# delldu/TransMVSNet

Hardware: AMD Instinct MI355X
Metric: depth maps/sec @ DTU 864x1152 N=5 (48/32/8 hyp); Abs depth L1 vs ref (higher is better)
Workload: dtype f32; 1 GPU; DTU 864x1152, N=5 views, cascade 48/32/8, B=1, hot path from FeatureNet outputs (FMT+pathway+stage glue+cost volume+CostRegNet+softmax/WTA); global_batch=1, parallelism=replica1, launch=hip_graph replay

## Files before the change

transmvsnet_amd/csrc/costreg.hip:

```cpp
#include "common.h"

namespace tmvs {

typedef float floatx4 __attribute__((ext_vector_type(4)));

template <int N>
struct VecN;
template <>
struct VecN<4> {
  float v[4];
  __device__ __forceinline__ void load(const float* p) {
    const float4 t = *reinterpret_cast<const float4*>(p);
    v[0] = t.x;
    v[1] = t.y;
    v[2] = t.z;
    v[3] = t.w;
  }
  __device__ __forceinline__ void zero() { v[0] = v[1] = v[2] = v[3] = 0.f; }
};
template <>
struct VecN<2> {
  float v[2];
  __device__ __forceinline__ void load(const float* p) {
    const float2 t = *reinterpret_cast<const float2*>(p);
// ... 515 lines not shown
      q[0] = make_float4(o[0], o[1], o[2], o[3]);
      q[1] = make_float4(o[4], o[5], o[6], o[7]);
    }
#pragma unroll
    for (int kh = 0; kh < 3; ++kh)
#pragma unroll
      for (int k = 0; k < 3; ++k) {
        win[0][kh][k] = win[1][kh][k];
        win[1][kh][k] = win[2][kh][k];
      }
  };
  float ra[3];
  load_raw(d0 - 1, ra);
  expand(ra, win[0]);
  load_raw(d0, ra);
  expand(ra, win[1]);
  load_raw(d0 + 1, ra);
  for (int d = d0; d < d1; ++d) step(d, ra);
}


template <int NR, typename Emit>
__device__ __forceinline__ void prob_walk_rows(__amdgpu_buffer_rsrc_t rx, int w, int h, int D, int H, int W, int d0,
                                               const float* __restrict__ wt, Emit emit) {
  constexpr int NL = NR + 2;
  d0 = __builtin_amdgcn_readfirstlane(d0);
  const unsigned offw = (unsigned)w < (unsigned)W ? (unsigned)w * 32u : kOffOut;
  auto load_plane = [&](int i, float4 (&o)[NL][2]) {
#pragma unroll
    for (int j = 0; j < NL; ++j) {
      const int ih = h - 1 + j;
      const unsigned offr = ((unsigned)i < (unsigned)D && (unsigned)ih < (unsigned)H)
                                ? ((unsigned)i * (unsigned)H + (unsigned)ih) * (unsigned)W * 32u
                                : kOffOut;
      const unsigned off = (offr + offw) | ((offr | offw) & kOffOut);
      const floatx4 u = buf_load_f32x4(rx, off);
      const floatx4 v = buf_load_f32x4(rx, off + 16u);
      o[j][0] = make_float4(u[0], u[1], u[2], u[3]);
      o[j][1] = make_float4(v[0], v[1], v[2], v[3]);
    }
  };
  float2_v c12[NR];
#pragma unroll
  for (int r = 0; r < NR; ++r) c12[r] = float2_v{0.f, 0.f};
  auto plane = [&](int i, const float4 (&p)[NL][2]) {
    float acc_next[NR];
#pragma unroll
    for (int r = 0; r < NR; ++r) acc_next[r] = 0.f;
#pragma unroll
    for (int kh = 0; kh < 3; ++kh) {
      int wo = kh * 72;
      asm volatile("" : "+s"(wo));
      const float* wk = wt + __builtin_amdgcn_readfirstlane(wo);
#pragma unroll
      for (int r = 0; r < NR; ++r) {
        const int j = r + kh;
        const float xc[8] = {p[j][0].x, p[j][0].y, p[j][0].z, p[j][0].w, p[j][1].x, p[j][1].y, p[j][1].z, p[j][1].w};
#pragma unroll
        for (int kw = 0; kw < 3; ++kw) {
#pragma unroll
          for (int c = 0; c < 8; ++c) {
            const float xv = kw == 0 ? lane_from_left(xc[c]) : kw == 1 ? xc[c] : lane_from_right(xc[c]);
            const float2_v wp = *reinterpret_cast<const float2_v*>(wk + 2 * (kw * 8 + c));
            acc_next[r] = fmaf(wk[48 + kw * 8 + c], xv, acc_next[r]);
            c12[r] = __builtin_elementwise_fma(wp, float2_v{xv, xv}, c12[r]);
          }
        }
        asm volatile("" : "+v"(acc_next[r]), "+v"(c12[r]));
      }
    }
#pragma unroll
    for (int r = 0; r < NR; ++r) {
      if (i - 1 >= d0) emit(r, i - 1, c12[r].y);
      c12[r] = float2_v{acc_next[r], c12[r].x};
    }
  };
  float4 pa[NL][2], pb[NL][2];
  load_plane(d0 - 1, pa);
#pragma unroll
  for (int j = 0; j < kDChunk + 2; j += 2) {
    const int i = d0 - 1 + j;
    load_plane(i + 1, pb);
    plane(i, pa);
    load_plane(i + 2, pa);
    plane(i + 1, pb);
  }
}

template <int NR>
__global__ __launch_bounds__(256) void prob_kernel(const float* __restrict__ x, float* __restrict__ y, int D, int H,
                                                   int W, const float* __restrict__ wt) {
  const int HW = H * W;
  const int nseg = (W + kProbCols - 1) / kProbCols, nrow = (H + 4 * NR - 1) / (4 * NR), ndc = (D + kDChunk - 1) / kDChunk;
  int lb = xcd_remap(blockIdx.x, gridDim.x);
  const int seg = lb % nseg;
  lb /= nseg;
  const int rowb = lb % nrow;
  lb /= nrow;
  const int dc = lb % ndc;
  const int n = lb / ndc;
  const int lane = threadIdx.x & 63;
  const int h = (rowb * 4 + (threadIdx.x >> 6)) * NR;
  if (h >= H) return;
  const int w = seg * kProbCols + lane - 1;
  const bool writes = lane >= 1 && lane <= kProbCols && w < W;
  const int d0 = dc * kDChunk, d1 = min(D, d0 + kDChunk);
  const __amdgpu_buffer_rsrc_t rx = raw_rsrc(x + (size_t)n * D * HW * 8, (unsigned)(D * HW * 32));
  float* yn = y + (size_t)n * D * HW + (size_t)h * W + w;
  prob_walk_rows<NR>(rx, w, h, D, H, W, d0, wt, [&](int r, int d, float v) {
    if (d < d1 && writes && h + r < H) yn[(size_t)d * HW + (size_t)r * W] = v;
  });
}

template <int D, int NR>
__global__ __launch_bounds__(64 * (D / kDChunk)) void prob_wta_rows_kernel(
    const float* __restrict__ x, const float* __restrict__ wt, const float* __restrict__ hyp, int H, int W, float lo,
    float hi, float* __restrict__ prob, float* __restrict__ depth, float* __restrict__ depth_raw,
    float* __restrict__ conf) {
  constexpr int NW = D / kDChunk;
  __shared__ float lg[NR][D * 64];
  const int HW = H * W;
  const int nseg = (W + kProbCols - 1) / kProbCols, nrow = (H + NR - 1) / NR;
  int lb = xcd_remap(blockIdx.x, gridDim.x);
  const int seg = lb % nseg;
  lb /= nseg;
  const int h0 = (lb % nrow) * NR;
  const int n = lb / nrow;
  const int lane = threadIdx.x & 63, wv = threadIdx.x >> 6;
  const int d0 = wv * kDChunk;
  const int w = seg * kProbCols + lane - 1;
  const bool writes = lane >= 1 && lane <= kProbCols && w < W;
  const __amdgpu_buffer_rsrc_t rx = raw_rsrc(x + (size_t)n * D * HW * 8, (unsigned)(D * HW * 32));
  prob_walk_rows<NR>(rx, w, h0, D, H, W, d0, wt, [&](int r, int d, float v) { lg[r][d * 64 + lane] = v; });
  __syncthreads();
  if (!writes) return;
  for (int r = wv; r < NR; r += NW) {
    const int h = h0 + r;
    if (h >= H) break;
    float xl[D];
#pragma unroll
    for (int d = 0; d < D; ++d) xl[d] = lg[r][d * 64 + lane];
    const size_t base = (size_t)n * D * HW + (size_t)h * W + w;
    float best;
    const int bi = softmax_first_max<D>(xl, [&](int d, float pr) { prob[base + (size_t)d * HW] = pr; }, best);
    const size_t o = (size_t)n * HW + (size_t)h * W + w;
    const float dr = hyp[base + (size_t)bi * HW];
    depth_raw[o] = dr;
    depth[o] = fminf(fmaxf(dr, lo), hi);
    conf[o] = best;
  }
}

template <int TD, int TH>
__global__ __launch_bounds__(256) __attribute__((amdgpu_waves_per_eu(2))) void conv3d_c16_kernel(const float* __restrict__ x, const float* __restrict__ wpk,
                                                         const float* __restrict__ alpha,
                                                         const float* __restrict__ shift, float* __restrict__ y, Geo g,
                                                         int ntiles) {
  constexpr int C = 16, PL = 4, NWV = 4, NBW = TD * TH / NWV, NTH = NWV * 64;
  static_assert(TD * TH % NWV == 0, "rows split evenly over the waves");
  constexpr int LW = 18, LH = TH + 2, LD = TD + 2, VST = 16;
  constexpr int NVOX = LD * LH * LW;
  constexpr int NLD = (NVOX * 4 + NTH - 1) / NTH;
  __shared__ __attribute__((aligned(16))) float tile[NVOX * VST];
  __shared__ __attribute__((aligned(16))) float wts[27 * 16 * 16];
  const int nws = (g.Wo + 15) / 16, nhs = (g.Ho + TH - 1) / TH, nds = (g.Do + TD - 1) / TD;
  const int lane = threadIdx.x & 63, wv = threadIdx.x >> 6;
  const int col = lane & 15, kgrp = lane >> 4;
  const int nxcd = gridDim.x >= 8 ? 8 : 1, per_xcd = gridDim.x / nxcd;
  const int xcd = blockIdx.x % nxcd, kx = blockIdx.x / nxcd;
  const int t_lo = (int)((long)ntiles * xcd / nxcd), t_hi = (int)((long)ntiles * (xcd + 1) / nxcd);
  if (kx >= per_xcd) return;
  struct TileCoord {
    int n, od0, oh0, ow0;
  };
  auto coord = [&](int t) {
    TileCoord c;
    c.ow0 = (t % nws) * 16;
    t /= nws;
    c.oh0 = (t % nhs) * TH;
    t /= nhs;
    c.od0 = (t % nds) * TD;
    c.n = t / nds;
    return c;
  };
  float4 pf[NLD];
  auto fetch = [&](int t) {
    const TileCoord c = coord(t);
    const size_t in_n = (size_t)c.n * g.Di * g.Hi * g.Wi;
#pragma unroll
    for (int k = 0; k < NLD; ++k) {
      const int idx = threadIdx.x + NTH * k;
      const int vox = idx >> 2, q = idx & 3;
      const int lw = vox % LW, rest = vox / LW, lh = rest % LH, ld = rest / LH;
      const int iw = c.ow0 - 1 + lw, ih = c.oh0 - 1 + lh, id = c.od0 - 1 + ld;
      pf[k] = make_float4(0.f, 0.f, 0.f, 0.f);
      if (vox < NVOX && (unsigned)iw < (unsigned)g.Wi && (unsigned)ih < (unsigned)g.Hi && (unsigned)id < (unsigned)g.Di)
        pf[k] = *reinterpret_cast<const float4*>(x + (in_n + ((size_t)id * g.Hi + ih) * g.Wi + iw) * C + 4 * q);
    }
  };
  auto commit = [&]() {
#pragma unroll
    for (int k = 0; k < NLD; ++k) {
      const int idx = threadIdx.x + NTH * k;
      const int vox = idx >> 2, q = idx & 3;
      if (vox < NVOX) *reinterpret_cast<float4*>(tile + vox * VST + 4 * (q ^ ((vox >> 1) & 3))) = pf[k];
    }
  };
  for (int idx = threadIdx.x; idx < 27 * 16 * 4; idx += NTH) {
    const int q = idx & 3, row = (idx >> 2) & 15, tap = idx >> 6;
    const float4 v = *reinterpret_cast<const float4*>(wpk + ((size_t)tap * C + row) * C + 4 * q);
    *reinterpret_cast<float4*>(wts + (tap * 16 + row) * 16 + 4 * (q ^ ((row >> 1) & 3))) = v;
  }
  const float4 al = *reinterpret_cast<const float4*>(alpha + kgrp * 4);
  const float4 sh = *reinterpret_cast<const float4*>(shift + kgrp * 4);
  int t = t_lo + kx;
  if (t < t_hi) {
    fetch(t);
    commit();
  }
  __syncthreads();
  for (; t < t_hi; t += per_xcd) {
    const TileCoord c = coord(t);
    const int tn = t + per_xcd;
    if (tn < t_hi) fetch(tn);
    floatx4 acc[NBW];
#pragma unroll
    for (int r = 0; r < NBW; ++r) acc[r] = floatx4{0.f, 0.f, 0.f, 0.f};
#pragma unroll
    for (int tap = 0; tap < 27; ++tap) {
      const int kd = tap / 9, kh = (tap / 3) % 3, kw = tap % 3;
      VecN<PL> a;
      a.load(wts + (tap * 16 + col) * 16 + 4 * (kgrp ^ ((col >> 1) & 3)));
      VecN<PL> b[NBW];
#pragma unroll
      for (int r = 0; r < NBW; ++r) {
        const int rr = wv * NBW + r;
        const int odl = rr / TH, ohl = rr - odl * TH;
        const int lvox = ((odl + kd) * LH + ohl + kh) * LW + col + kw;
        b[r].load(tile + lvox * VST + 4 * (kgrp ^ ((lvox >> 1) & 3)));
      }
#pragma unroll
      for (int j = 0; j < PL; ++j)
#pragma unroll
        for (int r = 0; r < NBW; ++r)
          acc[r] = __builtin_amdgcn_mfma_f32_16x16x4f32(a.v[j], b[r].v[j], acc[r], 0, 0, 0);
      if (tap % (NBW > 2 ? 3 : 9) == (NBW > 2 ? 2 : 8)) __builtin_amdgcn_sched_barrier(0);
    }
    const int ow = c.ow0 + col;
    const size_t out_n = (size_t)c.n * g.Do * g.Ho * g.Wo;
#pragma unroll
    for (int r = 0; r < NBW; ++r) {
      const int rr = wv * NBW + r;
      const int od = c.od0 + rr / TH, oh = c.oh0 + rr % TH;
      if (ow >= g.Wo || od >= g.Do || oh >= g.Ho) continue;
      float4 o;
      o.x = act(fmaf(acc[r][0], al.x, sh.x), g.lo);
      o.y = act(fmaf(acc[r][1], al.y, sh.y), g.lo);
      o.z = act(fmaf(acc[r][2], al.z, sh.z), g.lo);
      o.w = act(fmaf(acc[r][3], al.w, sh.w), g.lo);
      *reinterpret_cast<float4*>(y + (out_n + ((size_t)od * g.Ho + oh) * g.Wo + ow) * C + kgrp * 4) = o;
    }
    __syncthreads();
    if (tn < t_hi) commit();
    __syncthreads();
  }
}

template <typename K>
static int persistent_grid(K kernel, long ntiles) {
  struct Entry {
    const void* fn;
    int dev, cap;
  };
  static Entry cache[16];
  static int used = 0;
  int dev = 0;
  hipGetDevice(&dev);
  for (int i = 0; i < used; ++i)
    if (cache[i].fn == (const void*)kernel && cache[i].dev == dev) return (int)std::min<long>(ntiles, cache[i].cap);
  int cus = 0, per = 0;
  hipDeviceGetAttribute(&cus, hipDeviceAttributeMultiprocessorCount, dev);
  hipOccupancyMaxActiveBlocksPerMultiprocessor(&per, kernel, 256, 0);
  const int cap = std::max(8, cus * std::max(per, 1));
  if (used < 16) cache[used++] = Entry{(const void*)kernel, dev, cap};
  return (int)std::min<long>(ntiles, cap);
}

template <int TD, int TH>
static int launch_conv_c16(const float* x, const float* w, const float* al, const float* sh, float* y, int B,
                           const Geo& g, hipStream_t st) {
  const long ntiles = (long)B * ((g.Do + TD - 1) / TD) * ((g.Ho + TH - 1) / TH) * ((g.Wo + 15) / 16);
  const int grid = persistent_grid(conv3d_c16_kernel<TD, TH>, ntiles);
  hipLaunchKernelGGL((conv3d_c16_kernel<TD, TH>), dim3(grid), dim3(256), 0, st, x, w, al, sh, y, g, (int)ntiles);
  TMVS_CHECK_LAUNCH();
  return TMVS_OK;
}

template <int TD, int TH>
__global__ __launch_bounds__(256) __attribute__((amdgpu_waves_per_eu(1))) void conv3d_s2c8_tile_kernel(const float* __restrict__ x,
                                                               const float* __restrict__ wpk,
                                                               const float* __restrict__ alpha,
                                                               const float* __restrict__ shift, float* __restrict__ y,
                                                               Geo g, int ntiles) {
  constexpr int CIN = 8, COUT = 16, NWV = 4, NBW = TD * TH / NWV, NTH = NWV * 64;
  static_assert(TD * TH % NWV == 0, "rows split evenly over the waves");
  constexpr int LW = 33, LH = 2 * TH + 1, LD = 2 * TD + 1, SW = 17;
  constexpr int NROW = LD * LH, NQ = NROW * LW * 2;
  constexpr int NLD = (NQ + NTH - 1) / NTH;
  __shared__ __attribute__((aligned(16))) float tile[NROW * 2 * SW * 8];
  __shared__ __attribute__((aligned(16))) float wts[28 * 16 * 8];
  const int nws = (g.Wo + 15) / 16, nhs = (g.Ho + TH - 1) / TH, nds = (g.Do + TD - 1) / TD;
  const int lane = threadIdx.x & 63, wv = threadIdx.x >> 6;
  const int col = lane & 15, kgrp = lane >> 4;
  const int half = kgrp & 1, side = kgrp >> 1;
  const int nxcd = gridDim.x >= 8 ? 8 : 1, per_xcd = gridDim.x / nxcd;
  const int xcd = blockIdx.x % nxcd, kx = blockIdx.x / nxcd;
  const int t_lo = (int)((long)ntiles * xcd / nxcd), t_hi = (int)((long)ntiles * (xcd + 1) / nxcd);
  if (kx >= per_xcd) return;
  struct TileCoord {
    int n, od0, oh0, ow0;
  };
  auto coord = [&](int t) {
    TileCoord c;
    c.ow0 = (t % nws) * 16;
    t /= nws;
    c.oh0 = (t % nhs) * TH;
    t /= nhs;
    c.od0 = (t % nds) * TD;
    c.n = t / nds;
    return c;
  };
  float4 pf[NLD];
  auto fetch = [&](int t) {
    const TileCoord c = coord(t);
    const size_t in_n = (size_t)c.n * g.Di * g.Hi * g.Wi;
#pragma unroll
    for (int k = 0; k < NLD; ++k) {
      const int idx = threadIdx.x + NTH * k;
      const int q = idx & 1, v = idx >> 1;
      const int lw = v % LW, row = v / LW, lh = row % LH, ld = row / LH;
      const int iw = 2 * c.ow0 - 1 + lw, ih = 2 * c.oh0 - 1 + lh, id = 2 * c.od0 - 1 + ld;
      pf[k] = make_float4(0.f, 0.f, 0.f, 0.f);
      if (idx < NQ && (unsigned)iw < (unsigned)g.Wi && (unsigned)ih < (unsigned)g.Hi && (unsigned)id < (unsigned)g.Di)
        pf[k] = *reinterpret_cast<const float4*>(x + (in_n + ((size_t)id * g.Hi + ih) * g.Wi + iw) * CIN + 4 * q);
    }
  };
  auto commit = [&]() {
#pragma unroll
    for (int k = 0; k < NLD; ++k) {
      const int idx = threadIdx.x + NTH * k;
      const int q = idx & 1, v = idx >> 1;
      const int lw = v % LW, row = v / LW;
      if (idx < NQ) *reinterpret_cast<float4*>(tile + ((row * 2 + (lw & 1)) * SW + (lw >> 1)) * 8 + 4 * q) = pf[k];
    }
  };
  for (int idx = threadIdx.x; idx < 28 * 16 * 2; idx += NTH) {
    const int q = idx & 1, row = (idx >> 1) & 15, tap = idx >> 5;
    const float4 v = tap < 27 ? *reinterpret_cast<const float4*>(wpk + ((size_t)tap * COUT + row) * CIN + 4 * q)
                              : make_float4(0.f, 0.f, 0.f, 0.f);
    *reinterpret_cast<float4*>(wts + (tap * 16 + row) * 8 + 4 * q) = v;
  }
  const int co = kgrp * 4;
  const float4 al = *reinterpret_cast<const float4*>(alpha + co);
  const float4 sh = *reinterpret_cast<const float4*>(shift + co);
  int t = t_lo + kx;
  if (t < t_hi) {
    fetch(t);
    commit();
  }
  __syncthreads();
  for (; t < t_hi; t += per_xcd) {
    const TileCoord c = coord(t);
    const int tn = t + per_xcd;
    if (tn < t_hi) fetch(tn);
    floatx4 acc[NBW];
#pragma unroll
    for (int r = 0; r < NBW; ++r) acc[r] = floatx4{0.f, 0.f, 0.f, 0.f};
#pragma unroll
    for (int pr = 0; pr < 14; ++pr) {
      const int tap = 2 * pr + side;
      const int tp = tap < 27 ? tap : 26;
      const int kd = tp / 9, kh = (tp / 3) % 3, kw = tp % 3;
      const float4 a = *reinterpret_cast<const float4*>(wts + (tap * 16 + col) * 8 + 4 * half);
      float4 b[NBW];
#pragma unroll
      for (int r = 0; r < NBW; ++r) {
        const int rr = wv * NBW + r;
        const int odl = rr / TH, ohl = rr - odl * TH;
        const int row = (2 * odl + kd) * LH + 2 * ohl + kh;
        b[r] = *reinterpret_cast<const float4*>(tile + ((row * 2 + (kw & 1)) * SW + col + (kw >> 1)) * 8 + 4 * half);
      }
#pragma unroll
      for (int r = 0; r < NBW; ++r) acc[r] = __builtin_amdgcn_mfma_f32_16x16x4f32(a.x, b[r].x, acc[r], 0, 0, 0);
#pragma unroll
      for (int r = 0; r < NBW; ++r) acc[r] = __builtin_amdgcn_mfma_f32_16x16x4f32(a.y, b[r].y, acc[r], 0, 0, 0);
#pragma unroll
      for (int r = 0; r < NBW; ++r) acc[r] = __builtin_amdgcn_mfma_f32_16x16x4f32(a.z, b[r].z, acc[r], 0, 0, 0);
#pragma unroll
      for (int r = 0; r < NBW; ++r) acc[r] = __builtin_amdgcn_mfma_f32_16x16x4f32(a.w, b[r].w, acc[r], 0, 0, 0);
    }
    const int ow = c.ow0 + col;
    const size_t out_n = (size_t)c.n * g.Do * g.Ho * g.Wo;
#pragma unroll
    for (int r = 0; r < NBW; ++r) {
      const int rr = wv * NBW + r;
      const int od = c.od0 + rr / TH, oh = c.oh0 + rr % TH;
      if (ow >= g.Wo || od >= g.Do || oh >= g.Ho) continue;
      float4 o;
      o.x = act(fmaf(acc[r][0], al.x, sh.x), g.lo);
      o.y = act(fmaf(acc[r][1], al.y, sh.y), g.lo);
      o.z = act(fmaf(acc[r][2], al.z, sh.z), g.lo);
      o.w = act(fmaf(acc[r][3], al.w, sh.w), g.lo);
      *reinterpret_cast<float4*>(y + (out_n + ((size_t)od * g.Ho + oh) * g.Wo + ow) * COUT + co) = o;
    }
    __syncthreads();
    if (tn < t_hi) commit();
    __syncthreads();
  }
}

template <int TD, int TH>
static int launch_conv_s2c8_tile(const float* x, const float* w, const float* al, const float* sh, float* y, int B,
                                 const Geo& g, hipStream_t st) {
  const long ntiles = (long)B * ((g.Do + TD - 1) / TD) * ((g.Ho + TH - 1) / TH) * ((g.Wo + 15) / 16);
  const int grid = persistent_grid(conv3d_s2c8_tile_kernel<TD, TH>, ntiles);
  hipLaunchKernelGGL((conv3d_s2c8_tile_kernel<TD, TH>), dim3(grid), dim3(256), 0, st, x, w, al, sh, y, g, (int)ntiles);
  TMVS_CHECK_LAUNCH();
  return TMVS_OK;
}

template <int TD_, int TH_, int MBB_, int WS_>
struct LdsTile {
  static constexpr int TD = TD_, TH = TH_, MBB = MBB_, WS = WS_;
};

template <int CIN, int COUT, int S, typename T, bool KDSKIP = false, bool TAPOUT = false>
static int launch_conv(const float* x, const float* w, const float* al, const float* sh, float* y, int B,
                       const Geo& g, hipStream_t st) {
  constexpr int MG = ((COUT + 15) / 16) / T::MBB;
  const long nblk = (long)B * ((g.Do + T::TD - 1) / T::TD) * ((g.Ho + T::TH - 1) / T::TH) * ((g.Wo + 15) / 16) * MG;
  hipLaunchKernelGGL((conv3d_lds_kernel<CIN, COUT, S, T::TD, T::TH, T::MBB, T::WS, KDSKIP, TAPOUT>),
                     dim3((unsigned)nblk), dim3(256), 0, st, x, w, al, sh, y, g);
  TMVS_CHECK_LAUNCH();
  return TMVS_OK;
}

template <int TDI, int THI>
__global__ __launch_bounds__(256) __attribute__((amdgpu_waves_per_eu(4, 4))) void deconv3d_c8_kernel(const float* __restrict__ x, const float* __restrict__ wpk,
                                                          const float* __restrict__ alpha,
                                                          const float* __restrict__ shift,
                                                          const float* __restrict__ skip, float* __restrict__ y,
                                                          Geo g, int ntiles) {
  constexpr int CIN = 16, COUT = 8, PL = 4;
  constexpr int NBW = TDI * THI / 4;
  constexpr int LW = 17, LH = THI + 1, LD = TDI + 1, VST = 16;
  constexpr int NVOX = LD * LH * LW;
  constexpr int NLD = (NVOX * 4 + 255) / 256;
  static_assert((TDI * THI) % 4 == 0, "tile");
  __shared__ __attribute__((aligned(16))) float tile[2][NVOX * VST];
  __shared__ __attribute__((aligned(16))) float wts[27 * 8 * 16];
  __shared__ __attribute__((aligned(16))) float ep[4][32 * 8];

  const int nws = (g.Wi + 15) / 16, nhs = (g.Hi + THI - 1) / THI, nds = (g.Di + TDI - 1) / TDI;
  const int lane = threadIdx.x & 63, wv = threadIdx.x >> 6;
  const int col = lane & 15, kgrp = lane >> 4;
  const int nxcd = gridDim.x >= 8 ? 8 : 1, per_xcd = gridDim.x / nxcd;
  const int xcd = blockIdx.x % nxcd, kx = blockIdx.x / nxcd;
  const int t_lo = (int)((long)ntiles * xcd / nxcd), t_hi = (int)((long)ntiles * (xcd + 1) / nxcd);
  if (kx >= per_xcd) return;

  struct TileCoord {
    int n, md0, mh0, mw0;
  };
  auto coord = [&](int t) {
    TileCoord c;
    c.mw0 = (t % nws) * 16;
    t /= nws;
    c.mh0 = (t % nhs) * THI;
    t /= nhs;
    c.md0 = (t % nds) * TDI;
    c.n = t / nds;
    return c;
  };
  float4 pf[NLD];
  auto fetch = [&](int t) {
    const TileCoord c = coord(t);
    const size_t in_n = (size_t)c.n * g.Di * g.Hi * g.Wi;
#pragma unroll
    for (int k = 0; k < NLD; ++k) {
      const int idx = threadIdx.x + 256 * k;
      const int vox = idx >> 2, q = idx & 3;
      const int lw = vox % LW, rest = vox / LW, lh = rest % LH, ld = rest / LH;
      const int iw = c.mw0 + lw, ih = c.mh0 + lh, id = c.md0 + ld;
      pf[k] = make_float4(0.f, 0.f, 0.f, 0.f);
      if (vox < NVOX && iw < g.Wi && ih < g.Hi && id < g.Di)
        pf[k] = *reinterpret_cast<const float4*>(x + (in_n + ((size_t)id * g.Hi + ih) * g.Wi + iw) * CIN + 4 * q);
    }
  };
  auto commit = [&](float* buf) {
#pragma unroll
    for (int k = 0; k < NLD; ++k) {
      const int idx = threadIdx.x + 256 * k;
      const int vox = idx >> 2, q = idx & 3;
      if (vox < NVOX) *reinterpret_cast<float4*>(buf + vox * VST + 4 * (q ^ ((vox >> 1) & 3))) = pf[k];
    }
  };

  for (int idx = threadIdx.x; idx < 27 * 8 * 4; idx += 256) {
    const int q = idx & 3, row = (idx >> 2) & 7, tap = idx >> 5;
    const float4 v = *reinterpret_cast<const float4*>(wpk + ((size_t)tap * COUT + row) * CIN + 4 * q);
    *reinterpret_cast<float4*>(wts + (tap * 8 + row) * 16 + 4 * (q ^ ((row >> 1) & 3))) = v;
  }
  const int co = col & 7;
  const bool hi = col >= 8;
  float* eb = ep[wv];
  const int cq = 4 * (kgrp & 1);
  const float4 al = *reinterpret_cast<const float4*>(alpha + cq);
  const float4 sh = *reinterpret_cast<const float4*>(shift + cq);
  auto wfrag = [&](int tap, VecN<PL>& a) { a.load(wts + (tap * 8 + co) * 16 + 4 * (kgrp ^ ((co >> 1) & 3))); };

  int t = t_lo + kx;
  if (t < t_hi) {
    fetch(t);
    commit(tile[0]);
  }
  __syncthreads();
  for (int it = 0; t < t_hi; t += per_xcd, ++it) {
    const float* cur = tile[it & 1];
    const TileCoord c = coord(t);
    const int tn = t + per_xcd;
    if (tn < t_hi) fetch(tn);
    const size_t out_n = (size_t)c.n * g.Do * g.Ho * g.Wo;
    const int ow = 2 * c.mw0 + (lane >> 1);
    const size_t plane = (size_t)g.Ho * g.Wo * 8, row = (size_t)g.Wo * 8;
    float4 sk[NBW][4];
    size_t oo[NBW];
    bool ok[NBW];
#pragma unroll
    for (int r = 0; r < NBW; ++r) {
      const int rr = wv * NBW + r;
      const int md = c.md0 + rr / THI, mh = c.mh0 + rr % THI;
      ok[r] = md < g.Di && mh < g.Hi && ow < 2 * g.Wi;
      oo[r] = (out_n + ((size_t)(2 * md) * g.Ho + 2 * mh) * g.Wo + ow) * 8 + (lane & 1) * 4;
#pragma unroll
      for (int pdh = 0; pdh < 4; ++pdh)
        sk[r][pdh] = (ok[r] && skip) ? *reinterpret_cast<const float4*>(skip + oo[r] + (pdh >> 1) * plane + (pdh & 1) * row)
                           : make_float4(0.f, 0.f, 0.f, 0.f);
    }
    floatx4 acc[NBW][4];
#pragma unroll
    for (int r = 0; r < NBW; ++r)
#pragma unroll
      for (int q = 0; q < 4; ++q) acc[r][q] = floatx4{0.f, 0.f, 0.f, 0.f};
#pragma unroll
    for (int pdh = 0; pdh < 4; ++pdh) {
      const int pd = pdh >> 1, ph = pdh & 1;
#pragma unroll
      for (int td = 0; td < 1 + pd; ++td)
#pragma unroll
        for (int th = 0; th < 1 + ph; ++th) {
          const int kd = pd ? (td ? 2 : 0) : 1, od_off = (pd && !td) ? 1 : 0;
          const int kh = ph ? (th ? 2 : 0) : 1, oh_off = (ph && !th) ? 1 : 0;
          const int tap_base = kd * 9 + kh * 3;
          VecN<PL> a1, a2;
          wfrag(tap_base + (hi ? 2 : 1), a1);
          if (hi)
            wfrag(tap_base + 0, a2);
          else
            a2.zero();
#pragma unroll
          for (int r = 0; r < NBW; ++r) {
            const int rr = wv * NBW + r;
            const int mdl = rr / THI, mhl = rr - mdl * THI;
            const int lv = ((mdl + od_off) * LH + mhl + oh_off) * LW + col;
            VecN<PL> b1, b2;
            b1.load(cur + lv * VST + 4 * (kgrp ^ ((lv >> 1) & 3)));
            b2.load(cur + (lv + 1) * VST + 4 * (kgrp ^ (((lv + 1) >> 1) & 3)));
#pragma unroll
            for (int j = 0; j < PL; ++j)
              acc[r][pdh] = __builtin_amdgcn_mfma_f32_16x16x4f32(a1.v[j], b1.v[j], acc[r][pdh], 0, 0, 0);
#pragma unroll
            for (int j = 0; j < PL; ++j)
              acc[r][pdh] = __builtin_amdgcn_mfma_f32_16x16x4f32(a2.v[j], b2.v[j], acc[r][pdh], 0, 0, 0);
          }
          __builtin_amdgcn_sched_barrier(0);
        }
    }
#pragma unroll
    for (int r = 0; r < NBW; ++r)
#pragma unroll
      for (int pdh = 0; pdh < 4; ++pdh) {
        const floatx4 a = acc[r][pdh];
        *reinterpret_cast<float4*>(eb + (2 * col + (kgrp >> 1)) * 8 + cq) =
            make_float4(act(fmaf(a[0], al.x, sh.x), g.lo), act(fmaf(a[1], al.y, sh.y), g.lo), act(fmaf(a[2], al.z, sh.z), g.lo),
                        act(fmaf(a[3], al.w, sh.w), g.lo));
        __builtin_amdgcn_wave_barrier();
        const float4 v = *reinterpret_cast<const float4*>(eb + lane * 4);
        __builtin_amdgcn_wave_barrier();
        const float4 sv = sk[r][pdh];
        if (ok[r])
          *reinterpret_cast<float4*>(y + oo[r] + (pdh >> 1) * plane + (pdh & 1) * row) =
              make_float4(sv.x + v.x, sv.y + v.y, sv.z + v.z, sv.w + v.w);
      }
    if (tn < t_hi) commit(tile[(it + 1) & 1]);
    __syncthreads();
  }
}

template <int TDI, int THI>
static int launch_deconv_c8(const float* x, const float* w, const float* al, const float* sh, const float* skip,
                            float* y, int B, const Geo& g, hipStream_t st) {
  const long ntiles = (long)B * ((g.Di + TDI - 1) / TDI) * ((g.Hi + THI - 1) / THI) * ((g.Wi + 15) / 16);
  const long grid = persistent_grid(deconv3d_c8_kernel<TDI, THI>, ntiles);
  hipLaunchKernelGGL((deconv3d_c8_kernel<TDI, THI>), dim3((unsigned)grid), dim3(256), 0, st, x, w, al, sh, skip, y, g,
                     (int)ntiles);
  TMVS_CHECK_LAUNCH();
  return TMVS_OK;
}

template <int CIN, int COUT, int TDI, int THI, int MBB>
static int launch_deconv(const float* x, const float* w, const float* al, const float* sh, const float* skip,
                         float* y, int B, const Geo& g, hipStream_t st) {
  constexpr int MG = ((COUT + 15) / 16) / MBB;
  const long nblk = (long)B * ((g.Di + TDI - 1) / TDI) * ((g.Hi + THI - 1) / THI) * ((g.Wi + 15) / 16) * MG;
  hipLaunchKernelGGL((deconv3d_lds_kernel<CIN, COUT, TDI, THI, MBB>), dim3((unsigned)nblk), dim3(256), 0, st, x, w,
                     al, sh, skip, y, g);
  TMVS_CHECK_LAUNCH();
  return TMVS_OK;
}

static int conv_dispatch(const float* x, int B, int cin, int d, int h, int w, const float* wpk, const float* al,
                         const float* sh, int cout, int stride, float* y, hipStream_t st, float lo = 0.f) {
  Geo g;
  g.lo = lo;
  g.Di = d;
  g.Hi = h;
  g.Wi = w;
  if (stride == 1) {
    g.Do = d;
    g.Ho = h;
    g.Wo = w;
  } else {
    g.Do = (d - 1) / 2 + 1;
    g.Ho = (h - 1) / 2 + 1;
    g.Wo = (w - 1) / 2 + 1;
  }
  if ((long long)d * h * w * cin * 4 >= (1LL << 31)) return TMVS_ERR_SHAPE;
  constexpr int kKdSkipMaxDo = 2;
  const bool kdskip = g.Do <= kKdSkipMaxDo;
  constexpr bool KD = true, TAPOUT = true;
  using Conv3Tile = LdsTile<2, 2, 2, 2>;
  using Conv4Tile = LdsTile<2, 2, 2, 2>;
  using Conv4TileKd = LdsTile<2, 4, 2, 1>;
  using Conv5Tile = LdsTile<1, 2, 4, 4>;
  using Conv6Tile = LdsTile<1, 2, 4, 4>;
  int (*launch)(const float*, const float*, const float*, const float*, float*, int, const Geo&, hipStream_t) = nullptr;
  if (stride == 1) {
    if (cin == 16 && cout == 16)
      launch = launch_conv_c16<2, 4>;
    else if (cin == 32 && cout == 32)
      launch = kdskip ? launch_conv<32, 32, 1, Conv4TileKd, KD> : launch_conv<32, 32, 1, Conv4Tile>;
    else if (cin == 64 && cout == 64)
      launch = kdskip ? launch_conv<64, 64, 1, Conv6Tile, KD> : launch_conv<64, 64, 1, Conv6Tile>;
  } else {
    if (cin == 8 && cout == 16)
      launch = launch_conv_s2c8_tile<2, 2>;
    else if (cin == 16 && cout == 32)
      launch = kdskip ? launch_conv<16, 32, 2, Conv3Tile, KD> : launch_conv<16, 32, 2, Conv3Tile>;
    else if (cin == 32 && cout == 64)
      launch = launch_conv<32, 64, 2, Conv5Tile, false, TAPOUT>;
  }
  return launch ? launch(x, wpk, al, sh, y, B, g, st) : TMVS_ERR_SHAPE;
}

static int deconv_dispatch(const float* x, int B, int cin, int d, int h, int w, const float* wpk, const float* al,
                           const float* sh, int cout, const float* skip, float* y, hipStream_t st, float lo = 0.f) {
  Geo g;
  g.lo = lo;
  g.Di = d;
  g.Hi = h;
  g.Wi = w;
  g.Do = 2 * d;
  g.Ho = 2 * h;
  g.Wo = 2 * w;
  const bool even = g.Di % 2 == 0;
  int (*launch)(const float*, const float*, const float*, const float*, const float*, float*, int, const Geo&,
                hipStream_t) = nullptr;
  if (cin == 64 && cout == 32)
    launch = even ? launch_deconv<64, 32, 2, 2, 1> : launch_deconv<64, 32, 1, 4, 1>;
  else if (cin == 32 && cout == 16)
    launch = even ? launch_deconv<32, 16, 2, 2, 1> : launch_deconv<32, 16, 1, 4, 1>;
  else if (cin == 16 && cout == 8)
    launch = even ? launch_deconv_c8<2, 2> : launch_deconv_c8<1, 4>;
  return launch ? launch(x, wpk, al, sh, skip, y, B, g, st) : TMVS_ERR_SHAPE;
}


}

using namespace tmvs;

extern "C" int tmvs_conv3d_bn_relu(const float* x, int batch, int cin, int d, int h, int w, const float* wpk,
                                   const float* alpha, const float* shift, int cout, int stride, float* y,
                                   void* stream) {
  if (!x || !wpk || !alpha || !shift || !y || batch <= 0 || d <= 0 || h <= 0 || w <= 0) return TMVS_ERR_ARG;
  if (stride != 1 && stride != 2) return TMVS_ERR_ARG;
  return conv_dispatch(x, batch, cin, d, h, w, wpk, alpha, shift, cout, stride, y, (hipStream_t)stream);
}

extern "C" int tmvs_deconv3d_bn_relu_add(const float* x, int batch, int cin, int d, int h, int w, const float* wpk,
                                         const float* alpha, const float* shift, int cout, const float* skip,
                                         float* y, void* stream) {
  if (!x || !wpk || !alpha || !shift || !skip || !y || batch <= 0 || d <= 0 || h <= 0 || w <= 0)
    return TMVS_ERR_ARG;
  return deconv_dispatch(x, batch, cin, d, h, w, wpk, alpha, shift, cout, skip, y, (hipStream_t)stream);
}

static int launch_prob(const float* x, float* y, int batch, int D, int H, int W, const float* wt, hipStream_t st) {
  constexpr int NR = 1;
  const dim3 grid((unsigned)(((W + kProbCols - 1) / kProbCols) * ((H + 4 * NR - 1) / (4 * NR)) * batch *
                             ((D + kDChunk - 1) / kDChunk)));
  hipLaunchKernelGGL(prob_kernel<NR>, grid, dim3(256), 0, st, x, y, D, H, W, wt);
  TMVS_CHECK_LAUNCH();
  return TMVS_OK;
}

__device__ float kUnitAlpha[64] = {1.f, 1.f, 1.f, 1.f, 1.f, 1.f, 1.f, 1.f, 1.f, 1.f, 1.f, 1.f, 1.f, 1.f, 1.f, 1.f,
                                   1.f, 1.f, 1.f, 1.f, 1.f, 1.f, 1.f, 1.f, 1.f, 1.f, 1.f, 1.f, 1.f, 1.f, 1.f, 1.f,
                                   1.f, 1.f, 1.f, 1.f, 1.f, 1.f, 1.f, 1.f, 1.f, 1.f, 1.f, 1.f, 1.f, 1.f, 1.f, 1.f,
                                   1.f, 1.f, 1.f, 1.f, 1.f, 1.f, 1.f, 1.f, 1.f, 1.f, 1.f, 1.f, 1.f, 1.f, 1.f, 1.f};
__device__ float kZeroShift[64];

extern "C" int tmvs_conv3d_mfma(const float* x, int batch, int cin, int d, int h, int w, const float* wpk, int cout,
                                int stride, int transposed, const float* skip, float* y, void* stream) {
  if (!x || !wpk || !y || batch <= 0 || d <= 0 || h <= 0 || w <= 0) return TMVS_ERR_ARG;
  if (transposed ? stride != 2 : (stride != 1 && stride != 2)) return TMVS_ERR_ARG;
  if (skip && !transposed) return TMVS_ERR_ARG;
  int dev = 0;
  if (hipGetDevice(&dev) != hipSuccess || dev < 0 || dev >= 64) return TMVS_ERR_HIP;
  static const float* unit[64][2];
  if (!unit[dev][0]) {
    void *a, *b;
    if (hipGetSymbolAddress(&a, HIP_SYMBOL(kUnitAlpha)) != hipSuccess ||
        hipGetSymbolAddress(&b, HIP_SYMBOL(kZeroShift)) != hipSuccess)
      return TMVS_ERR_HIP;
    unit[dev][1] = (const float*)b;
    unit[dev][0] = (const float*)a;
  }
  const float *al = unit[dev][0], *sh = unit[dev][1];
  const float lo = -__builtin_huge_valf();
  hipStream_t st = (hipStream_t)stream;
  if (!transposed && stride == 1 && cin == 1 && cout == 8) {
    if ((long long)d * h * w * 32 >= (1LL << 31)) return TMVS_ERR_SHAPE;
    const dim3 grid((unsigned)(((w + kProbCols - 1) / kProbCols) * ((h + 3) / 4) * batch * ((d + kDChunk - 1) / kDChunk)));
    hipLaunchKernelGGL(conv0_kernel, grid, dim3(256), 0, st, x, y, d, h, w, wpk, al, sh, lo);
    TMVS_CHECK_LAUNCH();
    return TMVS_OK;
  }
  if (!transposed && stride == 1 && cin == 8 && cout == 1) {
    if ((long long)d * h * w * 32 >= (1LL << 31)) return TMVS_ERR_SHAPE;
    return launch_prob(x, y, batch, d, h, w, wpk, st);
  }
  if (transposed) return deconv_dispatch(x, batch, cin, d, h, w, wpk, al, sh, cout, skip, y, st, lo);
  return conv_dispatch(x, batch, cin, d, h, w, wpk, al, sh, cout, stride, y, st, lo);
}

// ... 125 lines not shown
```

Measured before the change: 299.9 depth_maps/s.

## Raise conv3d occupancy by trimming LDS and using buffer loads/stores

The c16 conv kernel moves the last two weight taps from LDS into registers so its LDS use fits three workgroups per CU, and it pins waves_per_eu to 3. Both c16 and s2c8 kernels switch global tile fetches to buffer loads with out-of-bounds offsets replacing branches, and prefetch unconditionally. The s2c8 kernel changes its LDS row stride and uses a buffer store for output. An env-gated residency log is added to the grid sizing. The aim is more resident waves to hide latency, at the cost of register pressure under the tighter waves_per_eu cap.

After: 302.0 depth_maps/s (median of 6 runs). No clear change (+0.7%).

```diff
diff --git a/transmvsnet_amd/csrc/costreg.hip b/transmvsnet_amd/csrc/costreg.hip
--- a/transmvsnet_amd/csrc/costreg.hip
+++ b/transmvsnet_amd/csrc/costreg.hip
@@ -691,7 +691,7 @@
 }
 
 template <int TD, int TH>
-__global__ __launch_bounds__(256) __attribute__((amdgpu_waves_per_eu(2))) void conv3d_c16_kernel(const float* __restrict__ x, const float* __restrict__ wpk,
+__global__ __launch_bounds__(256) __attribute__((amdgpu_waves_per_eu(3, 3))) void conv3d_c16_kernel(const float* __restrict__ x, const float* __restrict__ wpk,
                                                          const float* __restrict__ alpha,
                                                          const float* __restrict__ shift, float* __restrict__ y, Geo g,
                                                          int ntiles) {
@@ -700,8 +700,10 @@
   constexpr int LW = 18, LH = TH + 2, LD = TD + 2, VST = 16;
   constexpr int NVOX = LD * LH * LW;
   constexpr int NLD = (NVOX * 4 + NTH - 1) / NTH;
+  constexpr int NREG = 2, NLT = 27 - NREG;
   __shared__ __attribute__((aligned(16))) float tile[NVOX * VST];
-  __shared__ __attribute__((aligned(16))) float wts[27 * 16 * 16];
+  __shared__ __attribute__((aligned(16))) float wts[NLT * 16 * 16];
+  static_assert(sizeof(tile) + sizeof(wts) <= 42 * 1280, "three workgroups per CU");
   const int nws = (g.Wo + 15) / 16, nhs = (g.Ho + TH - 1) / TH, nds = (g.Do + TD - 1) / TD;
   const int lane = threadIdx.x & 63, wv = threadIdx.x >> 6;
   const int col = lane & 15, kgrp = lane >> 4;
@@ -722,19 +724,21 @@
     c.n = t / nds;
     return c;
   };
+  const uint32_t in_bytes = (uint32_t)g.Di * g.Hi * g.Wi * C * 4;
   float4 pf[NLD];
   auto fetch = [&](int t) {
-    const TileCoord c = coord(t);
-    const size_t in_n = (size_t)c.n * g.Di * g.Hi * g.Wi;
+    const bool live = t < t_hi;
+    const TileCoord c = coord(live ? t : t_lo);
+    const Buf xb(x + (size_t)c.n * g.Di * g.Hi * g.Wi * C, in_bytes);
 #pragma unroll
     for (int k = 0; k < NLD; ++k) {
       const int idx = threadIdx.x + NTH * k;
       const int vox = idx >> 2, q = idx & 3;
       const int lw = vox % LW, rest = vox / LW, lh = rest % LH, ld = rest / LH;
       const int iw = c.ow0 - 1 + lw, ih = c.oh0 - 1 + lh, id = c.od0 - 1 + ld;
-      pf[k] = make_float4(0.f, 0.f, 0.f, 0.f);
-      if (vox < NVOX && (unsigned)iw < (unsigned)g.Wi && (unsigned)ih < (unsigned)g.Hi && (unsigned)id < (unsigned)g.Di)
-        pf[k] = *reinterpret_cast<const float4*>(x + (in_n + ((size_t)id * g.Hi + ih) * g.Wi + iw) * C + 4 * q);
+      const bool ok = live && vox < NVOX && (unsigned)iw < (unsigned)g.Wi && (unsigned)ih < (unsigned)g.Hi &&
+                      (unsigned)id < (unsigned)g.Di;
+      pf[k] = xb.ld4(ok ? (((id * g.Hi + ih) * g.Wi + iw) * C + 4 * q) * 4 : Buf::kOOB);
     }
   };
   auto commit = [&]() {
@@ -745,23 +749,24 @@
       if (vox < NVOX) *reinterpret_cast<float4*>(tile + vox * VST + 4 * (q ^ ((vox >> 1) & 3))) = pf[k];
     }
   };
-  for (int idx = threadIdx.x; idx < 27 * 16 * 4; idx += NTH) {
+  for (int idx = threadIdx.x; idx < NLT * 16 * 4; idx += NTH) {
     const int q = idx & 3, row = (idx >> 2) & 15, tap = idx >> 6;
     const float4 v = *reinterpret_cast<const float4*>(wpk + ((size_t)tap * C + row) * C + 4 * q);
     *reinterpret_cast<float4*>(wts + (tap * 16 + row) * 16 + 4 * (q ^ ((row >> 1) & 3))) = v;
   }
+  VecN<PL> areg[NREG];
+#pragma unroll
+  for (int j = 0; j < NREG; ++j) areg[j].load(wpk + ((size_t)(NLT + j) * C + col) * C + 4 * kgrp);
   const float4 al = *reinterpret_cast<const float4*>(alpha + kgrp * 4);
   const float4 sh = *reinterpret_cast<const float4*>(shift + kgrp * 4);
   int t = t_lo + kx;
-  if (t < t_hi) {
-    fetch(t);
-    commit();
-  }
+  fetch(t);
+  commit();
   __syncthreads();
   for (; t < t_hi; t += per_xcd) {
     const TileCoord c = coord(t);
     const int tn = t + per_xcd;
-    if (tn < t_hi) fetch(tn);
+    fetch(tn);
     floatx4 acc[NBW];
 #pragma unroll
     for (int r = 0; r < NBW; ++r) acc[r] = floatx4{0.f, 0.f, 0.f, 0.f};
@@ -769,7 +774,10 @@
     for (int tap = 0; tap < 27; ++tap) {
       const int kd = tap / 9, kh = (tap / 3) % 3, kw = tap % 3;
       VecN<PL> a;
-      a.load(wts + (tap * 16 + col) * 16 + 4 * (kgrp ^ ((col >> 1) & 3)));
+      if (tap < NLT)
+        a.load(wts + (tap * 16 + col) * 16 + 4 * (kgrp ^ ((col >> 1) & 3)));
+      else
+        a = areg[tap >= NLT ? tap - NLT : 0];
       VecN<PL> b[NBW];
 #pragma unroll
       for (int r = 0; r < NBW; ++r) {
@@ -806,7 +814,7 @@
 }
 
 template <typename K>
-static int persistent_grid(K kernel, long ntiles) {
+static int persistent_grid(K kernel, long ntiles, const char* name) {
   struct Entry {
     const void* fn;
     int dev, cap;
@@ -821,6 +829,8 @@
   hipDeviceGetAttribute(&cus, hipDeviceAttributeMultiprocessorCount, dev);
   hipOccupancyMaxActiveBlocksPerMultiprocessor(&per, kernel, 256, 0);
   const int cap = std::max(8, cus * std::max(per, 1));
+  if (const char* e = getenv("TMVS_LOG_RESIDENCY"); e && e[0] == '1')
+    fprintf(stderr, "tmvs: %s: %d workgroups per CU x %d CUs\n", name, per, cus);
   if (used < 16) cache[used++] = Entry{(const void*)kernel, dev, cap};
   return (int)std::min<long>(ntiles, cap);
 }
@@ -829,7 +839,7 @@
 static int launch_conv_c16(const float* x, const float* w, const float* al, const float* sh, float* y, int B,
                            const Geo& g, hipStream_t st) {
   const long ntiles = (long)B * ((g.Do + TD - 1) / TD) * ((g.Ho + TH - 1) / TH) * ((g.Wo + 15) / 16);
-  const int grid = persistent_grid(conv3d_c16_kernel<TD, TH>, ntiles);
+  const int grid = persistent_grid(conv3d_c16_kernel<TD, TH>, ntiles, "conv3d_c16_kernel");
   hipLaunchKernelGGL((conv3d_c16_kernel<TD, TH>), dim3(grid), dim3(256), 0, st, x, w, al, sh, y, g, (int)ntiles);
   TMVS_CHECK_LAUNCH();
   return TMVS_OK;
@@ -843,11 +853,12 @@
                                                                Geo g, int ntiles) {
   constexpr int CIN = 8, COUT = 16, NWV = 4, NBW = TD * TH / NWV, NTH = NWV * 64;
   static_assert(TD * TH % NWV == 0, "rows split evenly over the waves");
-  constexpr int LW = 33, LH = 2 * TH + 1, LD = 2 * TD + 1, SW = 17;
+  constexpr int LW = 33, LH = 2 * TH + 1, LD = 2 * TD + 1, SW = 17, RS = 33;
   constexpr int NROW = LD * LH, NQ = NROW * LW * 2;
   constexpr int NLD = (NQ + NTH - 1) / NTH;
-  __shared__ __attribute__((aligned(16))) float tile[NROW * 2 * SW * 8];
+  __shared__ __attribute__((aligned(16))) float tile[NROW * RS * 8];
   __shared__ __attribute__((aligned(16))) float wts[28 * 16 * 8];
+  static_assert(sizeof(tile) + sizeof(wts) <= 32 * 1280, "four workgroups per CU");
   const int nws = (g.Wo + 15) / 16, nhs = (g.Ho + TH - 1) / TH, nds = (g.Do + TD - 1) / TD;
   const int lane = threadIdx.x & 63, wv = threadIdx.x >> 6;
   const int col = lane & 15, kgrp = lane >> 4;
@@ -870,18 +881,20 @@
     return c;
   };
   float4 pf[NLD];
+  const uint32_t in_bytes = (uint32_t)g.Di * g.Hi * g.Wi * CIN * 4;
   auto fetch = [&](int t) {
-    const TileCoord c = coord(t);
-    const size_t in_n = (size_t)c.n * g.Di * g.Hi * g.Wi;
+    const bool live = t < t_hi;
+    const TileCoord c = coord(live ? t : t_lo);
+    const Buf xb(x + (size_t)c.n * g.Di * g.Hi * g.Wi * CIN, in_bytes);
 #pragma unroll
     for (int k = 0; k < NLD; ++k) {
       const int idx = threadIdx.x + NTH * k;
       const int q = idx & 1, v = idx >> 1;
       const int lw = v % LW, row = v / LW, lh = row % LH, ld = row / LH;
       const int iw = 2 * c.ow0 - 1 + lw, ih = 2 * c.oh0 - 1 + lh, id = 2 * c.od0 - 1 + ld;
-      pf[k] = make_float4(0.f, 0.f, 0.f, 0.f);
-      if (idx < NQ && (unsigned)iw < (unsigned)g.Wi && (unsigned)ih < (unsigned)g.Hi && (unsigned)id < (unsigned)g.Di)
-        pf[k] = *reinterpret_cast<const float4*>(x + (in_n + ((size_t)id * g.Hi + ih) * g.Wi + iw) * CIN + 4 * q);
+      const bool ok = live && idx < NQ && (unsigned)iw < (unsigned)g.Wi && (unsigned)ih < (unsigned)g.Hi &&
+                      (unsigned)id < (unsigned)g.Di;
+      pf[k] = xb.ld4(ok ? (((id * g.Hi + ih) * g.Wi + iw) * CIN + 4 * q) * 4 : Buf::kOOB);
     }
   };
   auto commit = [&]() {
@@ -890,7 +903,7 @@
       const int idx = threadIdx.x + NTH * k;
       const int q = idx & 1, v = idx >> 1;
       const int lw = v % LW, row = v / LW;
-      if (idx < NQ) *reinterpret_cast<float4*>(tile + ((row * 2 + (lw & 1)) * SW + (lw >> 1)) * 8 + 4 * q) = pf[k];
+      if (idx < NQ) *reinterpret_cast<float4*>(tile + (row * RS + (lw & 1) * SW + (lw >> 1)) * 8 + 4 * q) = pf[k];
     }
   };
   for (int idx = threadIdx.x; idx < 28 * 16 * 2; idx += NTH) {
@@ -903,15 +916,13 @@
   const float4 al = *reinterpret_cast<const float4*>(alpha + co);
   const float4 sh = *reinterpret_cast<const float4*>(shift + co);
   int t = t_lo + kx;
-  if (t < t_hi) {
-    fetch(t);
-    commit();
-  }
+  fetch(t);
+  if (t < t_hi) commit();
   __syncthreads();
   for (; t < t_hi; t += per_xcd) {
     const TileCoord c = coord(t);
     const int tn = t + per_xcd;
-    if (tn < t_hi) fetch(tn);
+    fetch(tn);
     floatx4 acc[NBW];
 #pragma unroll
     for (int r = 0; r < NBW; ++r) acc[r] = floatx4{0.f, 0.f, 0.f, 0.f};
@@ -927,7 +938,7 @@
         const int rr = wv * NBW + r;
         const int odl = rr / TH, ohl = rr - odl * TH;
         const int row = (2 * odl + kd) * LH + 2 * ohl + kh;
-        b[r] = *reinterpret_cast<const float4*>(tile + ((row * 2 + (kw & 1)) * SW + col + (kw >> 1)) * 8 + 4 * half);
+        b[r] = *reinterpret_cast<const float4*>(tile + (row * RS + (kw & 1) * SW + col + (kw >> 1)) * 8 + 4 * half);
       }
 #pragma unroll
       for (int r = 0; r < NBW; ++r) acc[r] = __builtin_amdgcn_mfma_f32_16x16x4f32(a.x, b[r].x, acc[r], 0, 0, 0);
@@ -939,18 +950,20 @@
       for (int r = 0; r < NBW; ++r) acc[r] = __builtin_amdgcn_mfma_f32_16x16x4f32(a.w, b[r].w, acc[r], 0, 0, 0);
     }
     const int ow = c.ow0 + col;
-    const size_t out_n = (size_t)c.n * g.Do * g.Ho * g.Wo;
+    const __amdgpu_buffer_rsrc_t yb = __builtin_amdgcn_make_buffer_rsrc(
+        y + (size_t)c.n * g.Do * g.Ho * g.Wo * COUT, (short)0, (int)((uint32_t)g.Do * g.Ho * g.Wo * COUT * 4), 0x00020000);
 #pragma unroll
     for (int r = 0; r < NBW; ++r) {
       const int rr = wv * NBW + r;
       const int od = c.od0 + rr / TH, oh = c.oh0 + rr % TH;
-      if (ow >= g.Wo || od >= g.Do || oh >= g.Ho) continue;
-      float4 o;
-      o.x = act(fmaf(acc[r][0], al.x, sh.x), g.lo);
-      o.y = act(fmaf(acc[r][1], al.y, sh.y), g.lo);
-      o.z = act(fmaf(acc[r][2], al.z, sh.z), g.lo);
-      o.w = act(fmaf(acc[r][3], al.w, sh.w), g.lo);
-      *reinterpret_cast<float4*>(y + (out_n + ((size_t)od * g.Ho + oh) * g.Wo + ow) * COUT + co) = o;
+      typedef unsigned int uintx4 __attribute__((ext_vector_type(4)));
+      uintx4 o;
+      o[0] = __float_as_uint(act(fmaf(acc[r][0], al.x, sh.x), g.lo));
+      o[1] = __float_as_uint(act(fmaf(acc[r][1], al.y, sh.y), g.lo));
+      o[2] = __float_as_uint(act(fmaf(acc[r][2], al.z, sh.z), g.lo));
+      o[3] = __float_as_uint(act(fmaf(acc[r][3], al.w, sh.w), g.lo));
+      const bool ok = ow < g.Wo && od < g.Do && oh < g.Ho;
+      __builtin_amdgcn_raw_buffer_store_b128(o, yb, ok ? (((od * g.Ho + oh) * g.Wo + ow) * COUT + co) * 4 : Buf::kOOB, 0, 0);
     }
     __syncthreads();
     if (tn < t_hi) commit();
@@ -962,7 +975,7 @@
 static int launch_conv_s2c8_tile(const float* x, const float* w, const float* al, const float* sh, float* y, int B,
                                  const Geo& g, hipStream_t st) {
   const long ntiles = (long)B * ((g.Do + TD - 1) / TD) * ((g.Ho + TH - 1) / TH) * ((g.Wo + 15) / 16);
-  const int grid = persistent_grid(conv3d_s2c8_tile_kernel<TD, TH>, ntiles);
+  const int grid = persistent_grid(conv3d_s2c8_tile_kernel<TD, TH>, ntiles, "conv3d_s2c8_tile_kernel");
   hipLaunchKernelGGL((conv3d_s2c8_tile_kernel<TD, TH>), dim3(grid), dim3(256), 0, st, x, w, al, sh, y, g, (int)ntiles);
   TMVS_CHECK_LAUNCH();
   return TMVS_OK;
@@ -1150,7 +1163,7 @@
 static int launch_deconv_c8(const float* x, const float* w, const float* al, const float* sh, const float* skip,
                             float* y, int B, const Geo& g, hipStream_t st) {
   const long ntiles = (long)B * ((g.Di + TDI - 1) / TDI) * ((g.Hi + THI - 1) / THI) * ((g.Wi + 15) / 16);
-  const long grid = persistent_grid(deconv3d_c8_kernel<TDI, THI>, ntiles);
+  const long grid = persistent_grid(deconv3d_c8_kernel<TDI, THI>, ntiles, "deconv3d_c8_kernel");
   hipLaunchKernelGGL((deconv3d_c8_kernel<TDI, THI>), dim3((unsigned)grid), dim3(256), 0, st, x, w, al, sh, skip, y, g,
                      (int)ntiles);
   TMVS_CHECK_LAUNCH();
```
